# pagmerek/frave

Hardware: AMD Instinct MI355X
Metric: Mpixels/s encode (transform+quant) at 4096x4096 (higher is better)
Workload: dtype u8->i32

## Files before the change

### frave_amd/csrc/fri_hip.cpp

```cpp
#include "fri_hip_internal.hpp"
#include "region_table.hpp"

#include <atomic>
#include <cstdio>
#include <cstdlib>
#include <mutex>
#include <new>
#include <optional>
#include <thread>

#include "search_scaffold.hpp"
#include "solve6.hpp"

using namespace fri;
using namespace fri::host;

void PlanDelete::operator()(fri_hip_plan *p) const { delete p; }

struct fri_hip_multi {
    std::vector<fri_hip_ctx *> ctxs;
    std::vector<fri_hip_plan *> plans;
};

namespace {
// ... 15 lines not shown
    std::vector<float> t(10 * 1024);
    for (int b = 0; b < 10; b++)
        for (uint32_t j = 0; j < 1024; j++) {
            const float x = (float)((j & 1u) ? (int32_t)(j + 1) / -2 : (int32_t)(j / 2));
            t[b * 1024 + j] = std::exp(-std::fabs(x - 0.0f) / width[b]) / (2.0f * width[b]);
        }
    return t;
}

struct Knobs {
    int band_rows = 0, cells_per_tile = 0, cells_per_wg = 0, target_wgs = 0, tile_bytes = 0;
    int ranks = 0;
    std::optional<int> strided_shares;
    std::optional<int> k1_wave;
    int k1_wave_band = 0, k1_wave_wgs = 0;
    bool has_rank_weights = false;
    float rank_weight[4] = {0, 0, 0, 0};
    bool pins_forward = false;
    int batch_share_tiles = 0;
    std::optional<int> inv_shared, inv_strided_shares;
    int inv_band_rows = 0;
    int pred_blocks = 0, hist_blocks = 0, trace = 0, k3_scan = 0;
    int k1_ablate = 0, k2_ablate = 0, k3_ablate = 0, k4_ablate = 0;
    std::optional<int> k1_cached_stores, k1_batch_shares, k4_older_eighths;
};

Knobs read_knobs() {
    Knobs k;
    const char *on = std::getenv("FRI_HIP_TUNING");
    if (!on || on[0] != '1' || on[1] != 0) return k;
    auto env = [](const char *name) { return std::getenv(name); };
    auto pin = [&](const char *name) {
        const char *s = env(name);
        k.pins_forward |= s != nullptr;
        return s;
    };
    auto opt = [](const char *s) { return s ? std::optional<int>(std::atoi(s)) : std::nullopt; };
    auto num = [&](const char *s) { return opt(s).value_or(0); };
    k.band_rows = num(pin("FRI_HIP_BAND_ROWS")), k.cells_per_tile = num(pin("FRI_HIP_CELLS_PER_TILE")), k.cells_per_wg = num(pin("FRI_HIP_CELLS_PER_WG"));
    k.target_wgs = num(pin("FRI_HIP_TARGET_WGS")), k.tile_bytes = num(pin("FRI_HIP_TILE_BYTES")), k.ranks = std::min(num(pin("FRI_HIP_RANKS")), 4);
    k.strided_shares = opt(pin("FRI_HIP_STRIDED_SHARES"));
    k.k1_wave = opt(pin("FRI_HIP_K1_WAVE"));
    k.k1_wave_band = num(pin("FRI_HIP_K1_WAVE_BAND")), k.k1_wave_wgs = num(pin("FRI_HIP_K1_WAVE_WGS"));
    if (const char *s = pin("FRI_HIP_RANK_WEIGHTS")) {
        float *w = k.rank_weight;
        k.has_rank_weights = std::sscanf(s, "%f,%f,%f,%f", &w[0], &w[1], &w[2], &w[3]) == 4;
    }
    k.batch_share_tiles = num(env("FRI_HIP_BATCH_SHARE_TILES"));
    k.inv_shared = opt(env("FRI_HIP_INV_SHARED")), k.inv_strided_shares = opt(env("FRI_HIP_INV_STRIDED_SHARES")), k.inv_band_rows = num(env("FRI_HIP_INV_BAND_ROWS"));
    k.pred_blocks = num(env("FRI_HIP_PRED_BLOCKS")), k.hist_blocks = num(env("FRI_HIP_HIST_BLOCKS")), k.trace = num(env("FRI_HIP_TRACE")), k.k3_scan = num(env("FRI_HIP_K3_SCAN"));
    k.k1_ablate = num(env("FRI_HIP_K1_ABLATE")), k.k2_ablate = num(env("FRI_HIP_K2_ABLATE")), k.k3_ablate = num(env("FRI_HIP_K3_ABLATE")), k.k4_ablate = num(env("FRI_HIP_K4_ABLATE"));
    k.k1_cached_stores = opt(env("FRI_HIP_K1_CACHED_STORES")), k.k1_batch_shares = opt(env("FRI_HIP_K1_BATCH_SHARES")), k.k4_older_eighths = opt(env("FRI_HIP_K4_OLDER_EIGHTHS"));
    return k;
}

int acquire_acc(fri_hip_plan *p, hipStream_t stream, uint32_t n_planes = 1) {
    fri_hip_ctx *c = p->ctx;
    HIP_TRY(c, hipSetDevice(c->device));
// ... 90 lines not shown
            HIP_TRY(c, hipMalloc((void **)s.d_oob.put(), 2 * C * sizeof(unsigned long long)));
            HIP_TRY(c, hipHostMalloc((void **)s.h_oob.put(), 2 * C * sizeof(unsigned long long), hipHostMallocDefault));
            HIP_TRY(c, hipMalloc((void **)s.d_params.put(), C * sizeof(PredictParams)));
            HIP_TRY(c, hipHostMalloc((void **)s.h_params.put(), C * sizeof(PredictParams), hipHostMallocDefault));
        }
    }
    return FRI_HIP_OK;
}


void fill_forward_tiling(DevicePlan &d, const Geometry &g) {
    d.n_tiles = (uint32_t)g.tiles.size(), d.n_wg = (uint32_t)g.wg_tiles.size() - 1, d.n_wg_batch = (uint32_t)g.wg_tiles_batch.size() - 1;
    d.lds_pitch = g.lds_pitch, d.lds_rows = g.lds_rows, d.cells_per_tile = g.cells_per_tile, d.max_tile_cells = g.max_tile_cells;
    d.max_wg_tiles = std::max(g.max_wg_tiles, g.max_wg_tiles_batch), d.max_wg_cells = g.max_wg_cells;
    d.n_wave_wg = g.wave_cells.empty() ? 0u : (uint32_t)g.wave_cells.size() - 1, d.max_wave_wg_cells = g.max_wave_wg_cells;
    if (g.wave_cells.empty()) d.wave_meta = nullptr, d.wave_cells = nullptr;
}
void fill_inverse_tiling(DevicePlan &d, const Geometry &g) {
    fill_forward_tiling(d, g);
    d.wg_tiles_batch = nullptr, d.n_wg_batch = 0, d.max_wg_tiles = g.max_wg_tiles;
    d.wave_meta = nullptr, d.wave_cells = nullptr, d.n_wave_wg = 0, d.max_wave_wg_cells = 0;
    d.inv_group = 1, d.inv_max_wg_tiles = g.max_wg_tiles, d.inv_max_wg_cells = g.max_wg_cells;
}

hipError_t upload_tiling(std::vector<DevMem<void>> &bufs, const Geometry &g, DevicePlan &d, bool inverse) {
    hipError_t e;
    if ((e = upload(bufs, g.tiles, d.tiles)) || (e = upload(bufs, g.tile_cells, d.tile_cells)) || (e = upload(bufs, g.tile_meta, d.tile_meta)) ||
        (e = upload(bufs, g.wg_tiles, d.wg_tiles)) || (!inverse && (e = upload(bufs, g.wg_tiles_batch, d.wg_tiles_batch))))
        return e;
    if (!inverse && !g.wave_cells.empty() && ((e = upload(bufs, g.wave_meta, d.wave_meta)) || (e = upload(bufs, g.wave_cells, d.wave_cells)))) return e;
    inverse ? fill_inverse_tiling(d, g) : fill_forward_tiling(d, g);
    return hipSuccess;
}

int fwd_resident(const Geometry &g, uint32_t channels) {
    DevicePlan d;
// ... 37 lines not shown

constexpr size_t kStridedMaxCells = 200000, kOwnInverseMaxCells = 400000;
constexpr size_t kInvListsMaxBytes = (size_t)256 << 20;

int choose_forward_tiling(uint32_t width, uint32_t height, uint32_t channels, std::optional<int> cus, const Knobs &k, Tiling &t) {
    TilingParams &tp = t.tp;
    tp.band_rows = k.band_rows;
    tp.cells_per_tile = k.cells_per_tile;
    tp.cells_per_wg = k.cells_per_wg;
    tp.batch_share_tiles = k.batch_share_tiles;
    tp.strided_shares = k.strided_shares ? *k.strided_shares > 0 : cus.has_value();
    if (!k.strided_shares && (size_t)width * height / kCell >= kStridedMaxCells) tp.strided_shares = false;
    if (tp.band_rows <= 0 && cus) tp.band_rows = 16;
    tp.tile_buffer_bytes = k.tile_bytes > 0 ? k.tile_bytes : (channels == 1 ? 4 : 6) * 256 * 16;
    set_ranks(tp, k.ranks > 0 ? k.ranks : 4, cus, k);
    if (k.k1_wave.value_or(0) > 0 && cus) tp.wave_ranks = std::min(k.k1_wave_wgs > 0 ? k.k1_wave_wgs : 4, fwd_wave_resident()), tp.wave_band_rows = std::max(k.k1_wave_band, 0);
    for (;;) {
        const std::string err = build_geometry(width, height, channels, tp, t.geo);
        if (!err.empty()) return err == "empty lattice" ? FRI_HIP_ERR_EMPTY_LATTICE : FRI_HIP_ERR_INVALID_ARGUMENT;
        const int resident = fwd_resident(t.geo, channels);
        const size_t F = t.geo.centers.size();
        if (!resident) {
            if (!shrink_tiling(tp, t.geo)) return FRI_HIP_ERR_INVALID_ARGUMENT;
        } else if (cus && !k.strided_shares && tp.strided_shares && F >= kStridedMaxCells) {
            tp.strided_shares = false;
        } else if (cus && k.ranks <= 0 && resident < tp.ranks) {
            set_ranks(tp, resident, cus, k);
        } else if (cus && !t.many_shares && k.target_wgs <= 0 && tp.cells_per_wg <= 0 && F >= 128 * (size_t)(*cus * tp.ranks)) {
            t.many_shares = true;
            tp.target_wgs = (int)(((F / 32 + 1023) / 1024) * 1024);
            for (int i = 0; i < 4; i++) tp.rank_weight[i] = i < tp.ranks ? 1.f : 0.f;
        } else {
            return FRI_HIP_OK;
        }
    }
}

bool choose_inverse_tiling(uint32_t width, uint32_t height, uint32_t channels, std::optional<int> cus, const Knobs &k, const Tiling &fwd, Tiling &inv) {
    if (!cus || (k.inv_shared ? *k.inv_shared > 0 : fwd.geo.centers.size() >= kOwnInverseMaxCells)) return false;
    TilingParams &ti = inv.tp;
    ti = fwd.tp;
    ti.wave_ranks = 0;
    set_ranks(ti, fwd.tp.ranks, cus, k);
    ti.band_rows = k.inv_band_rows > 0 ? k.inv_band_rows : (channels == 1 ? 32 : 16);
    ti.cells_per_tile = k.cells_per_tile;
    ti.cells_per_wg = 0;
    ti.target_wgs = *cus * ti.ranks;
    ti.strided_shares = k.inv_strided_shares ? *k.inv_strided_shares > 0 : k.strided_shares.value_or(1) > 0;
    for (int guard = 0; guard < 64; guard++) {
        if (!build_geometry(width, height, channels, ti, inv.geo).empty()) return false;
        if (fwd_resident(inv.geo, channels) && inv_fits(inv.geo, channels, false)) {
            build_inverse_lists(inv.geo, kInvListsMaxBytes);
            return inv.geo.inv_lists.empty() || inv_fits(inv.geo, channels, true);
        }
        if (!shrink_tiling(ti, inv.geo)) return false;
    }
    return false;
// ... 22 lines not shown
    return resident > 0 && resident >= c.tp.ranks;
}

hipError_t upload_forward_candidate(const fri_hip_plan *p, FwdTiling &c) {
    c.dev = p->dev;
    c.dev.k1_measuring = true;
    return upload_tiling(c.bufs, c.geo, c.dev, false);
}

void adopt_forward_tiling(fri_hip_plan *p, FwdTiling &c) {
    Geometry &g = p->geo;
    g.tiles.swap(c.geo.tiles), g.tile_cells.swap(c.geo.tile_cells), g.tile_meta.swap(c.geo.tile_meta), g.wg_tiles.swap(c.geo.wg_tiles), g.wg_tiles_batch.swap(c.geo.wg_tiles_batch);
    g.max_wg_tiles_batch = c.geo.max_wg_tiles_batch, g.lds_pitch = c.geo.lds_pitch, g.lds_rows = c.geo.lds_rows, g.band_rows = c.geo.band_rows, g.cells_per_tile = c.geo.cells_per_tile;
    g.cells_per_wg = c.geo.cells_per_wg, g.max_tile_cells = c.geo.max_tile_cells, g.max_wg_tiles = c.geo.max_wg_tiles, g.max_wg_cells = c.geo.max_wg_cells;
    g.wave_meta.swap(c.geo.wave_meta), g.wave_cells.swap(c.geo.wave_cells);
    g.wave_band_rows = c.geo.wave_band_rows, g.wave_ranks = c.geo.wave_ranks, g.max_wave_wg_cells = c.geo.max_wave_wg_cells;
    DevicePlan &d = p->dev;
    d.tiles = c.dev.tiles, d.tile_cells = c.dev.tile_cells, d.tile_meta = c.dev.tile_meta, d.wg_tiles = c.dev.wg_tiles, d.wg_tiles_batch = c.dev.wg_tiles_batch;
    d.wave_meta = c.dev.wave_meta, d.wave_cells = c.dev.wave_cells;
    fill_forward_tiling(d, g);
    d.inv_max_wg_tiles = d.max_wg_tiles, d.inv_max_wg_cells = d.max_wg_cells;
    for (auto &b : c.bufs) p->owned.push_back(std::move(b));
    c.bufs.clear();
    p->fwd_tp = c.tp;
    p->fwd_tiling_note = c.label;
}

std::string tiling_label(const TilingParams &tp, const Geometry &g) {
    char b[96];
    if (tp.wave_ranks > 0 && !g.wave_cells.empty()) std::snprintf(b, sizeof b, "wave/band%d/wg%d", g.wave_band_rows, g.wave_ranks);
    else std::snprintf(b, sizeof b, "%s/band%d/cells%d", tp.strided_shares ? "interleaved" : "contiguous", g.band_rows, g.cells_per_tile);
    std::string l = b;
    if (tp.rank_weight[0] > 0) {
        std::snprintf(b, sizeof b, "/w%.2f-%.2f", tp.rank_weight[0], tp.rank_weight[std::max(0, std::min(tp.ranks, 4) - 1)]);
        l += b;
    }
    return l;
}

struct TunedKey {
    int device;
    uint32_t w, h, c;
    bool operator==(const TunedKey &o) const { return device == o.device && w == o.w && h == o.h && c == o.c; }
};
std::mutex g_tuned_mu;
std::vector<std::pair<TunedKey, TilingParams>> g_tuned;

void adopt_cached_forward_tiling(fri_hip_plan *p) {
// ... 170 lines not shown
    if (!out) return FRI_HIP_ERR_INVALID_ARGUMENT;
    *out = nullptr;
    const StaticTables &st = static_tables();
    if (!st.error.empty() || !device_footprint_matches(st)) return FRI_HIP_ERR_INVALID_ARGUMENT;
    std::unique_ptr<fri_hip_plan, PlanDelete> plan(new (std::nothrow) fri_hip_plan);
    if (!plan) return FRI_HIP_ERR_OUT_OF_MEMORY;
    fri_hip_plan *p = plan.get();
    p->ctx = ctx;
    const Knobs k = read_knobs();
    const std::optional<int> cus = ctx ? std::optional<int>(ctx->cu_count) : std::nullopt;
    Tiling fwd, inv;
    if (int rc = choose_forward_tiling(width, height, channels, cus, k, fwd)) return rc;
    p->own_inverse_tiling = choose_inverse_tiling(width, height, channels, cus, k, fwd, inv);
    p->geo = std::move(fwd.geo);
    p->fwd_tp = fwd.tp;
    if (!p->geo.wave_cells.empty()) p->fwd_tiling_note = tiling_label(fwd.tp, p->geo) + " (pinned: FRI_HIP_K1_WAVE)";
    if (p->own_inverse_tiling) {
        p->geo_inv = std::move(inv.geo);
        std::vector<uint32_t>().swap(p->geo_inv.valid_mask), std::vector<int32_t>().swap(p->geo_inv.nbr_cells), std::vector<int32_t>().swap(p->geo_inv.pred_slots);
    } else {
        build_inverse_lists(p->geo, kInvListsMaxBytes);
    }
    if (!ctx) {
        p->dev.n_pred_tiles = p->geo.n_pred_tiles;
        p->dev.pred_blocks = (uint32_t)std::max(k.pred_blocks, 0), p->dev.hist_blocks = (uint32_t)std::max(k.hist_blocks, 0);
        p->dev.k4_older_eighths = k.k4_older_eighths.value_or(0);
        *out = plan.release();
        return FRI_HIP_OK;
    }
    if (hipSetDevice(ctx->device) != hipSuccess) return FRI_HIP_ERR_HIP;
    const Geometry &g = p->geo, &gi = p->inv_geo();
// ... 1035 lines not shown
    }
    for (uint32_t k = 1; k < n_streams; k++) {
        HIP_TRY(c, hipEventRecord(done[k], st[k]));
        HIP_TRY(c, hipStreamWaitEvent(st[0], done[k], 0));
    }
    HIP_TRY(c, hipEventRecord(e1, st[0]));
    HIP_TRY(c, hipEventSynchronize(e1));
    float ms = 0.f;
    HIP_TRY(c, hipEventElapsedTime(&ms, e0, e1));
    *mean_us = (double)ms * 1000.0 / iters;
    return FRI_HIP_OK;
}

static int tune_forward(fri_hip_plan *p, uint32_t launches, std::string &rep) {
    if (!p->fwd_tunable) {
        rep = "{\"tuned\": false, \"kept\": \"" + p->fwd_tiling_note + "\", \"why\": \"tiling pinned by the environment, shared with the inverse kernel, or a many-shares plan\"}";
        return FRI_HIP_OK;
    }
    fri_hip_ctx *c = p->ctx;
    HIP_TRY(c, hipSetDevice(c->device));
    if (!launches) launches = 96;
    const Geometry &g0 = p->geo;
    const bool rgb = g0.channels != 1;
    std::vector<std::unique_ptr<FwdTiling>> cand;
    auto add_tp = [&](const TilingParams &tp) {
        auto t = std::make_unique<FwdTiling>();
        t->tp = tp;
        if (t->tp.cells_per_tile < 0 || t->tp.band_rows < 0) return;
        if (!build_forward_candidate(p, *t)) return;
        t->label = tiling_label(t->tp, t->geo);
        for (const auto &o : cand)
// ... 108 lines not shown
            size_t b2 = best;
            for (size_t k : round2)
                if (cand[k]->us < cand[b2]->us) b2 = k;
            if (cand[b2]->us < cand[best]->us * 0.99) best = b2;
        }
    }
    if (!rgb && g0.width % 16 == 0) {
        const TilingParams w = cand[best]->tp;
        std::vector<size_t> round3{best};
        const size_t n0 = cand.size();
        for (int ranks : {4, 5})
            for (int band : {16, 32, 72, 96, 112, 128}) {
                if (ranks == 5 && band != 32 && band != 96) continue;
                TilingParams tp = w;
                tp.wave_ranks = ranks, tp.wave_band_rows = band;
                add_tp(tp);
                if (band >= (int)g0.height) break;
            }
        for (size_t k = n0; k < cand.size(); k++) {
            HIP_TRY(c, upload_forward_candidate(p, *cand[k]));
            round3.push_back(k);
        }
        if (round3.size() > 1) {
            HIP_TRY(c, measure(round3));
            size_t b3 = best;
            for (size_t k : round3)
                if (cand[k]->us < cand[b3]->us) b3 = k;
            if (cand[b3]->us < cand[best]->us * 0.985) best = b3;
        }
    }
    std::string xcd_note;
    if (hipMalloc((void **)d_stat.put(), 16 * sizeof(unsigned long long)) == hipSuccess) {
        unsigned long long h_stat[16];
        HIP_TRY(c, hipMemsetAsync(d_stat, 0, sizeof h_stat, stream));
        cand[best]->dev.k1_xcd_stat = d_stat;
        const hipError_t e_run = run(*cand[best], launches);
        cand[best]->dev.k1_xcd_stat = nullptr;
        HIP_TRY(c, e_run);
        HIP_TRY(c, hipStreamSynchronize(stream));
        HIP_TRY(c, hipMemcpy(h_stat, d_stat, sizeof h_stat, hipMemcpyDeviceToHost));
        for (int x = 0; x < 8; x++) {
            char b[32];
            std::snprintf(b, sizeof b, "%s%.2f", x ? " " : "", h_stat[2 * x + 1] ? (double)h_stat[2 * x] / (double)h_stat[2 * x + 1] / 100.0 : 0.0);
// ... 34 lines not shown
```

### frave_amd/csrc/geometry.cpp

```cpp
#include "geometry.hpp"

#include <algorithm>
#include <climits>
#include <cstdlib>
#include <cstring>
#include <deque>

namespace fri {

namespace {

constexpr Int2 kLiterals[11] = {{0, 1}, {-1, 1}, {2, 0}, {-3, -1}, {5, -1}, {1, 3}, {-11, -1}, {9, -5}, {13, 7}, {-31, 3}, {5, -17}};

inline Int2 add(Int2 a, Int2 b) { return {a.x + b.x, a.y + b.y}; }
inline Int2 sub(Int2 a, Int2 b) { return {a.x - b.x, a.y - b.y}; }
inline Int2 neg(Int2 a) { return {-a.x, -a.y}; }
inline int floor_div(int a, int b) { return (a >= 0) ? a / b : -((-a + b - 1) / b); }
inline int pos_mod(int a, int m) {
    int r = a % m;
    return r < 0 ? r + m : r;
}

struct LatticeBasis {
    Int2 zl, zmd;
// ... 140 lines not shown
        zmd = add(kLiterals[depth + 1], zl);
    }
    out[0] = zl;
    out[1] = sub(zl, zmd);
    out[2] = neg(zmd);
    out[3] = neg(zl);
    out[4] = sub(zmd, zl);
    out[5] = zmd;
}

static void build_wave_shares(const TilingParams &tp, Geometry &g) {
    const size_t F = g.centers.size();
    const int ranks = std::min(std::max(tp.wave_ranks, 1), 6), tile_ranks = std::min(std::max(tp.ranks, 1), 4);
    const int band_rows = tp.wave_band_rows > 0 ? tp.wave_band_rows : 16;
    const size_t cus = std::max<size_t>(1, (size_t)(tp.target_wgs > 0 ? tp.target_wgs : 1024) / tile_ranks);
    g.wave_band_rows = band_rows, g.wave_ranks = ranks;
    const int cy_min = g.centers.front().y;
    std::vector<int32_t> order(F);
    for (size_t k = 0; k < F; k++) order[k] = (int32_t)k;
    std::sort(order.begin(), order.end(), [&](int32_t l, int32_t r) {
        const int bl = (g.centers[l].y - cy_min) / band_rows, br = (g.centers[r].y - cy_min) / band_rows;
        if (bl != br) return bl < br;
        if (g.centers[l].x != g.centers[r].x) return g.centers[l].x < g.centers[r].x;
        return g.centers[l].y < g.centers[r].y;
    });
    g.wave_meta.resize(F);
    for (size_t k = 0; k < F; k++) g.wave_meta[k] = TileCell{g.centers[order[k]].x, g.centers[order[k]].y, order[k], g.interior[order[k]]};
    const size_t n_wg = std::max<size_t>(1, std::min(cus * ranks, (F + 1) / 2));
    const bool weighted = tp.rank_weight[0] > 0 && tp.rank_weight[tile_ranks - 1] > 0;
    auto weight = [&](size_t rank) {
        if (!weighted || ranks == 1) return 1.0;
        return (double)tp.rank_weight[0] + ((double)tp.rank_weight[tile_ranks - 1] - (double)tp.rank_weight[0]) * (double)rank / (double)(ranks - 1);
    };
    std::vector<double> cum(n_wg + 1, 0.0);
    const size_t q = n_wg >> 3, r = n_wg & 7;
    for (size_t x = 0, sh = 0; x < 8; x++) {
        const size_t n_x = q + (x < r ? 1 : 0);
        for (size_t idx = 0; idx < n_x; idx++, sh++) cum[sh + 1] = cum[sh] + weight(std::min<size_t>((idx * 8 + x) / cus, ranks - 1));
    }
    g.wave_cells.assign(n_wg + 1, 0);
    for (size_t sh = 0; sh <= n_wg; sh++) g.wave_cells[sh] = (int32_t)((double)F * cum[sh] / cum[n_wg] + 0.5);
    g.wave_cells[0] = 0;
    g.wave_cells[n_wg] = (int32_t)F;
    g.max_wave_wg_cells = 0;
    for (size_t sh = 1; sh <= n_wg; sh++) {
        g.wave_cells[sh] = (int32_t)std::min<size_t>(std::max<size_t>((size_t)g.wave_cells[sh], (size_t)g.wave_cells[sh - 1] + 1), F - (n_wg - sh));
        g.max_wave_wg_cells = std::max(g.max_wave_wg_cells, g.wave_cells[sh] - g.wave_cells[sh - 1]);
// ... 354 lines not shown
```

### frave_amd/csrc/geometry.hpp

```cpp
#pragma once
#include <cstdint>
#include <string>
#include <vector>

namespace fri {

struct Int2 {
    int32_t x, y;
};

constexpr int kDepth = 9;
constexpr int kCell = 1 << kDepth;
constexpr int kNbr = 8;

struct StaticTables {
    Int2 literals[11];
    Int2 leaf_off[kCell];
    uint16_t residue_lut[kCell];
    Int2 v9[6];
    Int2 nbr_delta[kNbr];
    uint16_t nbr_table[kCell][6];
    std::string error;
};
const StaticTables &static_tables();
// ... 23 lines not shown
    uint64_t n_valid_leaves = 0;
    std::vector<Int2> centers;
    std::vector<uint8_t> interior;
    std::vector<uint32_t> valid_mask;
    std::vector<int32_t> nbr_cells;
    std::vector<Tile> tiles;
    std::vector<int32_t> tile_cells;
    std::vector<TileCell> tile_meta;
    std::vector<int32_t> wg_tiles;
    std::vector<int32_t> wg_tiles_batch;
    int32_t max_wg_tiles_batch = 0;
    std::vector<TileCell> wave_meta;
    std::vector<int32_t> wave_cells;
    int32_t wave_band_rows = 0, wave_ranks = 0;
    int32_t max_wave_wg_cells = 0;
    std::vector<InvTileLists> inv_lists;
    std::vector<uint16_t> inv_quads, inv_dwords;
    std::vector<uint32_t> inv_parts;
    int32_t inv_rect_bytes = 0;
    int32_t lds_pitch = 0;
    int32_t lds_rows = 0;
    int32_t band_rows = 0, cells_per_tile = 0, cells_per_wg = 0;
    int32_t max_tile_cells = 0;
    int32_t max_wg_tiles = 0;
    int32_t max_wg_cells = 0;
    std::vector<int32_t> pred_slots;
    uint32_t n_pred_tiles = 0;
};

constexpr int32_t kPredSlotInterior = 0x40000000;
constexpr int kPredBlock = 4;
constexpr int kPredSide = kPredBlock + 2;
constexpr int kPredSlots = kPredSide * kPredSide;

struct TilingParams {
    int band_rows = 0, cells_per_tile = 0;
    int target_wgs = 0;
    int cells_per_wg = 0;
    float rank_weight[4] = {0, 0, 0, 0};
    int ranks = 4;
    int tile_buffer_bytes = 0;
    int batch_share_tiles = 0;
    int wave_ranks = 0, wave_band_rows = 0;
    bool strided_shares = false;
};

std::string build_geometry(uint32_t width, uint32_t height, uint32_t channels, const TilingParams &tp, Geometry &out);
void build_inverse_lists(Geometry &g, size_t max_bytes);

}
```

### frave_amd/csrc/k1_forward.hip

```cpp
#include "device_common.hpp"

namespace fri {
namespace {

constexpr int kFwdThreads = 256;
constexpr int kFwdWaves = kFwdThreads / 64;

constexpr int kMaxPairsPerWave = 2;
constexpr int kMaxItemsPerTile = 2 * kMaxPairsPerWave * kFwdWaves;
constexpr int kMaxChunksPerThread = 6;

struct FwdArgs {
    const uint8_t *pixels;
    size_t pixel_stride;
    int32_t *coefs;
    size_t coef_stride;
    const Tile *tiles;
    const TileCell *tile_meta;
    const int32_t *wg_tiles;
    uint32_t n_wg;
    int32_t width, height;
    uint32_t F;
    int32_t pitch;
    int32_t meta_off;
    int32_t buf_bytes;
    uint32_t cpr, cpr_magic;
    int32_t q_identity;
    int32_t ablate;
    unsigned long long *trace;
    unsigned long long *xcd_stat;
    QMatrix q;
};

__device__ __forceinline__ uint32_t pk_low(uint32_t l, uint32_t r, uint32_t x) { return __builtin_amdgcn_lerp(l, r, x >> 15); }
__device__ __forceinline__ void pk_pair(uint32_t l, uint32_t r, int &dA, int &dB, uint32_t &s) {
    s = pk_low(l, r, l - r);
    dA = (int)(l & 0xFFFFu) - (int)(r & 0xFFFFu);
    dB = (int)(l >> 16) - (int)(r >> 16);
}
__device__ __forceinline__ void unpack_x(uint32_t x, int &dA, int &dB) {
    dA = (int)(short)(x & 0xFFFFu);
    dB = (int)(x + 0x8000u) >> 16;
}
// ... 514 lines not shown

constexpr int kWavePitch = 160, kWaveRows = 21, kWaveItemBytes = 64;
constexpr int kWaveSlab = kWaveRows * kWavePitch;
constexpr int kWaveItemChunks = kWaveRows * 4;
constexpr int kWaveLoads = 3;
constexpr int kWaveLdsBytes = 2 * kFwdWaves * kWaveSlab;
constexpr int kWaveMaxWgCells = 64 * kFwdWaves;
typedef u32x4 __attribute__((address_space(3))) *LdsQuadPtr;

struct WaveChunks {
    int row[kWaveLoads], k16[kWaveLoads];
    bool item_b[kWaveLoads], used[kWaveLoads];
    uint32_t lds_off[kWaveLoads];
};

template <bool QID, bool MEASURE = false>
__global__ void __launch_bounds__(kFwdThreads) fwd_wave_kernel(const FwdArgs a) {
    __shared__ __attribute__((aligned(16))) uint8_t slabs[kWaveLdsBytes];
    const int tid = threadIdx.x, lane = tid & 63;
    const int wave = __builtin_amdgcn_readfirstlane(tid >> 6);
    const uint32_t wg = xcd_contiguous_share(blockIdx.x, a.n_wg);
    const int cb = a.wg_tiles[wg], ce = a.wg_tiles[wg + 1];
    const unsigned long long t_entry = a.xcd_stat ? wall_clock64() : 0ull;
    const int wg_pairs = (ce - cb + 1) >> 1;
    const int n_pairs = wg_pairs > wave ? (wg_pairs - wave + kFwdWaves - 1) / kFwdWaves : 0;
    if (n_pairs > 0) {
        const uint8_t *img = a.pixels + (size_t)blockIdx.y * a.pixel_stride;
        int32_t *coefs = a.coefs + (size_t)blockIdx.y * a.coef_stride;
        const int mine = cb + 2 * (wave + kFwdWaves * (lane >> 1)) + (lane & 1);
        const i32x4 rec = reinterpret_cast<const i32x4 *>(a.tile_meta)[min(mine, ce - 1)];
        const uint32_t slab0 = (uint32_t)(uintptr_t)(__attribute__((address_space(3))) uint8_t *)slabs + (uint32_t)wave * (2u * kWaveSlab);

        WaveChunks ch;
#pragma unroll
        for (int c = 0; c < kWaveLoads; c++) {
            const int s = lane + 64 * c;
            ch.used[c] = s < 2 * kWaveItemChunks;
            ch.item_b[c] = s >= kWaveItemChunks;
            const int w = ch.item_b[c] ? s - kWaveItemChunks : s;
            ch.row[c] = ch.used[c] ? w >> 2 : 0;
            ch.k16[c] = 16 * (w & 3);
// ... 13 lines not shown
            for (int c = 0; c < kWaveLoads; c++) {
                const int x = (ch.item_b[c] ? xB : xA) + ch.k16[c], y = (ch.item_b[c] ? cyB : cyA) - 8 + ch.row[c];
                const bool inside = wanted && ch.used[c] && (uint32_t)x < (uint32_t)a.width && (uint32_t)y < (uint32_t)a.height;
                st[c] = *reinterpret_cast<const u32x4 *>(img + (inside ? (uint32_t)y * (uint32_t)a.width + (uint32_t)x : 0u));
            }
        };
        auto commit = [&](uint32_t slab) {
#pragma unroll
            for (int c = 0; c < kWaveLoads; c++) *(LdsQuadPtr)(uintptr_t)(slab + ch.lds_off[c]) = st[c];
        };
        issue(0, true);
        commit(slab0);

        for (int i = 0; i < n_pairs; i++) {
            const uint32_t cur = slab0 + (uint32_t)(i & 1) * kWaveSlab, nxt = slab0 + (uint32_t)((i & 1) ^ 1) * kWaveSlab;
            issue(min(i + 1, n_pairs - 1), i + 1 < n_pairs);
            __builtin_amdgcn_s_setprio(3);
            const int cxA = __builtin_amdgcn_readlane(rec.x, 2 * i), cyA = __builtin_amdgcn_readlane(rec.y, 2 * i);
            const int cxB = __builtin_amdgcn_readlane(rec.x, 2 * i + 1), cyB = __builtin_amdgcn_readlane(rec.y, 2 * i + 1);
            const uint32_t offA = (uint32_t)__builtin_amdgcn_readlane(rec.z, 2 * i) * kCell, offB = (uint32_t)__builtin_amdgcn_readlane(rec.z, 2 * i + 1) * kCell;
            const int interior = __builtin_amdgcn_readlane(rec.w, 2 * i) & __builtin_amdgcn_readlane(rec.w, 2 * i + 1);
            const bool store_b = cb + 2 * (wave + kFwdWaves * i) + 1 < ce;
            const int baseA = (int)cur + ((cxA - 15) & 15), baseB = (int)cur + kWaveItemBytes + ((cxB - 15) & 15);
            const int wbA[3] = {baseA + wo[0], baseA + wo[1], baseA + wo[2]}, wbB[3] = {baseB + wo[0], baseB + wo[1], baseB + wo[2]};
            uint32_t wA[3], wB[3], maskA = 0xFFu, maskB = 0xFFu;
            fetch_windows(wbA, wA);
            fetch_windows(wbB, wB);
            if (interior == 0) {
                maskA = maskB = 0;
#pragma unroll
// ... 16 lines not shown
            leaf[7] = pair_bytes<2>(wA[2], wB[2]);
            int resA[8], resB[8];
            fwd_wave_pk(leaf, lane, resA, resB);
            __builtin_amdgcn_s_setprio(1);
            uint32_t valid = 0xFFFFFFFFu;
            if (interior == 0) valid = validity_tree_pk(maskA | (maskB << 16), lane);
            commit(nxt);
            __builtin_amdgcn_s_setprio(0);
            if (__builtin_amdgcn_readfirstlane(valid == 0xFFFFFFFFu ? 1 : 0) && __all(valid == 0xFFFFFFFFu)) {
                store_item<0, false, QID, true>(coefs, offA, lane, resA, valid, a);
                if (store_b) store_item<1, false, QID, true>(coefs, offB, lane, resB, valid, a);
            } else {
                store_item<0, true, QID, true>(coefs, offA, lane, resA, valid, a);
                if (store_b) store_item<1, true, QID, true>(coefs, offB, lane, resB, valid, a);
            }
        }
    }
    if (a.xcd_stat && tid == 0) {
        const uint32_t xcc = __builtin_amdgcn_s_getreg((3 << 11) | 20) & 7u;
        (void)__hip_atomic_fetch_add(a.xcd_stat + 2 * xcc, wall_clock64() - t_entry, __ATOMIC_RELAXED, __HIP_MEMORY_SCOPE_AGENT);
        (void)__hip_atomic_fetch_add(a.xcd_stat + 2 * xcc + 1, 1ull, __ATOMIC_RELAXED, __HIP_MEMORY_SCOPE_AGENT);
    }
}


}

const void *pick_forward_ycbcr(bool edge, bool fast, bool small, bool qid, bool plain, bool measure, bool c16);
#ifndef FRI_K1_YCBCR_INSTANCES

static size_t fwd_meta_offset(const DevicePlan &p) { return ((size_t)p.lds_pitch * p.lds_rows + 15) & ~(size_t)15; }
static size_t fwd_buf_bytes(const DevicePlan &p) { return fwd_meta_offset(p) + (size_t)p.max_tile_cells * sizeof(TileCell); }
// ... 44 lines not shown
    a.cpr_magic = (uint32_t)(((1ull << 32) + a.cpr - 1) / a.cpr);
    a.q = q;
    a.q_identity = 1;
    for (int i = 0; i <= 9; i++) a.q_identity &= (q.q[i] == 1);
    a.ablate = p.k1_ablate;
    a.trace = p.trace;
    a.xcd_stat = p.k1_xcd_stat;
    const size_t lds = fwd_lds_bytes(p);
    const dim3 grid(a.n_wg, n_images), block(kFwdThreads);
    const size_t img_bytes = (size_t)p.width * p.height * p.channels;
    const bool edge = (reinterpret_cast<uintptr_t>(pixels) & 15) || (img_bytes & 15) || (n_images > 1 && (pixel_stride & 15));
    const bool fast = !edge && (((size_t)p.width * p.channels) & 15) == 0;
    const bool small = fwd_chunks(p) <= 4 * (size_t)kFwdThreads;
    const bool rct = p.rct && p.channels == 3;
    const bool ycc = p.ycc && p.channels == 3;
    if (fast && !plain && !coefs16 && n_images < 8 && !p.trace && !p.k1_ablate && fwd_wave_fits(p)) {
        a.tile_meta = p.wave_meta;
        a.wg_tiles = p.wave_cells;
        a.n_wg = p.n_wave_wg;
        void (*wk)(FwdArgs) = a.q_identity ? (p.k1_measuring ? fwd_wave_kernel<true, true> : fwd_wave_kernel<true>) : fwd_wave_kernel<false>;
        (void)hipGetLastError();
        hipLaunchKernelGGL(wk, dim3(a.n_wg, n_images), block, 0, stream, a);
        return hipGetLastError();
    }
    void (*kern)(FwdArgs);
#define FRI_PICK_T(CH, E, FA, N, QI, R) (plain ? fwd_transform_quant_kernel<CH, E, FA, N, QI, false, false, false, R> : fwd_transform_quant_kernel<CH, E, FA, N, QI, true, false, false, R>)
#define FRI_PICK_Q(CH, E, FA, N, R) (a.q_identity ? FRI_PICK_T(CH, E, FA, N, true, R) : FRI_PICK_T(CH, E, FA, N, false, R))
#define FRI_PICK_N(CH, E, FA, R) (small ? FRI_PICK_Q(CH, E, FA, 4, R) : FRI_PICK_Q(CH, E, FA, kMaxChunksPerThread, R))
#define FRI_PICK(CH, R) (edge ? FRI_PICK_N(CH, true, false, R) : fast ? FRI_PICK_N(CH, false, true, R) : FRI_PICK_N(CH, false, false, R))
    kern = p.channels == 1 ? FRI_PICK(1, false) : rct ? FRI_PICK(3, true) : FRI_PICK(3, false);
    if (p.k1_measuring && !edge && !plain && a.q_identity) {
#define FRI_PICK_M(CH, R) (fast ? (small ? fwd_transform_quant_kernel<CH, false, true, 4, true, true, true, false, R> : fwd_transform_quant_kernel<CH, false, true, kMaxChunksPerThread, true, true, true, false, R>) \
                                : (small ? fwd_transform_quant_kernel<CH, false, false, 4, true, true, true, false, R> : fwd_transform_quant_kernel<CH, false, false, kMaxChunksPerThread, true, true, true, false, R>))
        kern = p.channels == 1 ? FRI_PICK_M(1, false) : rct ? FRI_PICK_M(3, true) : FRI_PICK_M(3, false);
#undef FRI_PICK_M
// ... 27 lines not shown
```

### frave_amd/csrc/kernels.hpp

```cpp
#pragma once
#include <hip/hip_runtime_api.h>

#include <cstddef>
#include <cstdint>

#include "geometry.hpp"

namespace fri {

struct DevicePlan {
    const Tile *tiles = nullptr;
    const int32_t *tile_cells = nullptr;
    const TileCell *tile_meta = nullptr;
    const int32_t *wg_tiles = nullptr;
    const int32_t *wg_tiles_batch = nullptr;
    uint32_t n_wg_batch = 0;
    uint32_t n_wg = 0;
    const TileCell *wave_meta = nullptr;
    const int32_t *wave_cells = nullptr;
    uint32_t n_wave_wg = 0;
    int32_t max_wave_wg_cells = 0;
    int32_t max_tile_cells = 0;
    bool covers_image = false;
    int32_t max_wg_tiles = 0;
    int32_t max_wg_cells = 0;
    int32_t inv_group = 1;
    int32_t inv_max_wg_tiles = 0, inv_max_wg_cells = 0;
    const Int2 *centers = nullptr;
    const uint8_t *interior = nullptr;
    const uint32_t *valid_mask = nullptr;
    const int32_t *nbr_cells = nullptr;
    const uint16_t *nbr_table = nullptr;
    const uint32_t *gather_off = nullptr;
    const uint16_t *pair_pos = nullptr;
    const uint16_t *heap_of_pos = nullptr;
    const uint32_t *halo_list = nullptr;
// ... 145 lines not shown

hipError_t launch_split_tiles_rgba(const uint8_t *rgba, uint32_t width, uint32_t height, uint32_t tile_w, uint32_t tile_h, bool clean, uint8_t *colour_tiles, uint8_t *alpha_tiles,
                                   hipStream_t stream);
hipError_t launch_merge_tiles_rgba_region(const uint8_t *colour_tiles, const uint8_t *alpha_tiles, uint32_t width, uint32_t height, uint32_t tile_w, uint32_t tile_h, uint32_t x,
                                          uint32_t y, uint32_t w, uint32_t h, uint8_t *region, hipStream_t stream);

void build_lf_deltas(const uint16_t *nbr_table, int8_t *out );
void build_gather_tables(const uint16_t *nbr_table, uint32_t *gather_off , uint16_t *pair_pos , uint16_t *heap_of_pos );
void build_halo_list(const uint16_t *nbr_table, const uint16_t *pair_pos, uint32_t *out );
size_t fwd_lds_bytes(const DevicePlan &p);
size_t inv_lds_bytes(const DevicePlan &p);
bool device_footprint_matches(const StaticTables &st);
bool fwd_plan_fits(const DevicePlan &p);
bool fwd_wave_fits(const DevicePlan &p);
int fwd_wave_resident();
constexpr size_t kInvListPad = 2048;
bool inv_plan_fits(const DevicePlan &p, bool with_lists);

}
```

Baseline: 936,700.

## Add paced wave-kernel variant and autotune pacing and wave rank weights

```diff
diff --git a/frave_amd/csrc/fri_hip.cpp b/frave_amd/csrc/fri_hip.cpp
--- a/frave_amd/csrc/fri_hip.cpp
+++ b/frave_amd/csrc/fri_hip.cpp
@@ -53,6 +53,7 @@
     std::optional<int> strided_shares;
     std::optional<int> k1_wave;
     int k1_wave_band = 0, k1_wave_wgs = 0;
+    int k1_wave_pace = 0;
     bool has_rank_weights = false;
     float rank_weight[4] = {0, 0, 0, 0};
     bool pins_forward = false;
@@ -81,6 +82,7 @@
     k.strided_shares = opt(pin("FRI_HIP_STRIDED_SHARES"));
     k.k1_wave = opt(pin("FRI_HIP_K1_WAVE"));
     k.k1_wave_band = num(pin("FRI_HIP_K1_WAVE_BAND")), k.k1_wave_wgs = num(pin("FRI_HIP_K1_WAVE_WGS"));
+    k.k1_wave_pace = num(pin("FRI_HIP_K1_WAVE_PACE"));
     if (const char *s = pin("FRI_HIP_RANK_WEIGHTS")) {
         float *w = k.rank_weight;
         k.has_rank_weights = std::sscanf(s, "%f,%f,%f,%f", &w[0], &w[1], &w[2], &w[3]) == 4;
@@ -201,12 +203,13 @@
     d.lds_pitch = g.lds_pitch, d.lds_rows = g.lds_rows, d.cells_per_tile = g.cells_per_tile, d.max_tile_cells = g.max_tile_cells;
     d.max_wg_tiles = std::max(g.max_wg_tiles, g.max_wg_tiles_batch), d.max_wg_cells = g.max_wg_cells;
     d.n_wave_wg = g.wave_cells.empty() ? 0u : (uint32_t)g.wave_cells.size() - 1, d.max_wave_wg_cells = g.max_wave_wg_cells;
+    d.wave_pace_ticks = g.wave_cells.empty() ? 0u : std::min((uint32_t)std::max(g.wave_pace_ticks, 0), kWavePaceMaxTicks);
     if (g.wave_cells.empty()) d.wave_meta = nullptr, d.wave_cells = nullptr;
 }
 void fill_inverse_tiling(DevicePlan &d, const Geometry &g) {
     fill_forward_tiling(d, g);
     d.wg_tiles_batch = nullptr, d.n_wg_batch = 0, d.max_wg_tiles = g.max_wg_tiles;
-    d.wave_meta = nullptr, d.wave_cells = nullptr, d.n_wave_wg = 0, d.max_wave_wg_cells = 0;
+    d.wave_meta = nullptr, d.wave_cells = nullptr, d.n_wave_wg = 0, d.max_wave_wg_cells = 0, d.wave_pace_ticks = 0;
     d.inv_group = 1, d.inv_max_wg_tiles = g.max_wg_tiles, d.inv_max_wg_cells = g.max_wg_cells;
 }
 
@@ -274,7 +277,9 @@
     if (tp.band_rows <= 0 && cus) tp.band_rows = 16;
     tp.tile_buffer_bytes = k.tile_bytes > 0 ? k.tile_bytes : (channels == 1 ? 4 : 6) * 256 * 16;
     set_ranks(tp, k.ranks > 0 ? k.ranks : 4, cus, k);
-    if (k.k1_wave.value_or(0) > 0 && cus) tp.wave_ranks = std::min(k.k1_wave_wgs > 0 ? k.k1_wave_wgs : 4, fwd_wave_resident()), tp.wave_band_rows = std::max(k.k1_wave_band, 0);
+    const bool wave_pinned = k.k1_wave ? *k.k1_wave > 0 : k.k1_wave_pace > 0;
+    if (wave_pinned && cus) tp.wave_ranks = std::min(k.k1_wave_wgs > 0 ? k.k1_wave_wgs : 4, fwd_wave_resident()), tp.wave_band_rows = std::max(k.k1_wave_band, 0);
+    if (wave_pinned && cus && k.k1_wave_pace > 0) tp.wave_pace_ticks = (int)std::min<uint32_t>((uint32_t)k.k1_wave_pace, kWavePaceMaxTicks);
     for (;;) {
         const std::string err = build_geometry(width, height, channels, tp, t.geo);
         if (!err.empty()) return err == "empty lattice" ? FRI_HIP_ERR_EMPTY_LATTICE : FRI_HIP_ERR_INVALID_ARGUMENT;
@@ -300,7 +305,7 @@
     if (!cus || (k.inv_shared ? *k.inv_shared > 0 : fwd.geo.centers.size() >= kOwnInverseMaxCells)) return false;
     TilingParams &ti = inv.tp;
     ti = fwd.tp;
-    ti.wave_ranks = 0;
+    ti.wave_ranks = 0, ti.wave_pace_ticks = 0;
     set_ranks(ti, fwd.tp.ranks, cus, k);
     ti.band_rows = k.inv_band_rows > 0 ? k.inv_band_rows : (channels == 1 ? 32 : 16);
     ti.cells_per_tile = k.cells_per_tile;
@@ -353,7 +358,7 @@
     g.max_wg_tiles_batch = c.geo.max_wg_tiles_batch, g.lds_pitch = c.geo.lds_pitch, g.lds_rows = c.geo.lds_rows, g.band_rows = c.geo.band_rows, g.cells_per_tile = c.geo.cells_per_tile;
     g.cells_per_wg = c.geo.cells_per_wg, g.max_tile_cells = c.geo.max_tile_cells, g.max_wg_tiles = c.geo.max_wg_tiles, g.max_wg_cells = c.geo.max_wg_cells;
     g.wave_meta.swap(c.geo.wave_meta), g.wave_cells.swap(c.geo.wave_cells);
-    g.wave_band_rows = c.geo.wave_band_rows, g.wave_ranks = c.geo.wave_ranks, g.max_wave_wg_cells = c.geo.max_wave_wg_cells;
+    g.wave_band_rows = c.geo.wave_band_rows, g.wave_ranks = c.geo.wave_ranks, g.max_wave_wg_cells = c.geo.max_wave_wg_cells, g.wave_pace_ticks = c.geo.wave_pace_ticks;
     DevicePlan &d = p->dev;
     d.tiles = c.dev.tiles, d.tile_cells = c.dev.tile_cells, d.tile_meta = c.dev.tile_meta, d.wg_tiles = c.dev.wg_tiles, d.wg_tiles_batch = c.dev.wg_tiles_batch;
     d.wave_meta = c.dev.wave_meta, d.wave_cells = c.dev.wave_cells;
@@ -367,10 +372,18 @@
 
 std::string tiling_label(const TilingParams &tp, const Geometry &g) {
     char b[96];
-    if (tp.wave_ranks > 0 && !g.wave_cells.empty()) std::snprintf(b, sizeof b, "wave/band%d/wg%d", g.wave_band_rows, g.wave_ranks);
+    const bool wave = tp.wave_ranks > 0 && !g.wave_cells.empty();
+    if (wave) std::snprintf(b, sizeof b, "wave/band%d/wg%d", g.wave_band_rows, g.wave_ranks);
     else std::snprintf(b, sizeof b, "%s/band%d/cells%d", tp.strided_shares ? "interleaved" : "contiguous", g.band_rows, g.cells_per_tile);
     std::string l = b;
-    if (tp.rank_weight[0] > 0) {
+    if (wave && g.wave_pace_ticks > 0) {
+        std::snprintf(b, sizeof b, "/pace%d", (g.wave_pace_ticks + 5) / 10);
+        l += b;
+    }
+    if (wave && tp.wave_weight[0] > 0) {
+        std::snprintf(b, sizeof b, "/w%.2f-%.2f", tp.wave_weight[0], tp.wave_weight[1]);
+        l += b;
+    } else if (tp.rank_weight[0] > 0) {
         std::snprintf(b, sizeof b, "/w%.2f-%.2f", tp.rank_weight[0], tp.rank_weight[std::max(0, std::min(tp.ranks, 4) - 1)]);
         l += b;
     }
@@ -571,7 +584,7 @@
     p->own_inverse_tiling = choose_inverse_tiling(width, height, channels, cus, k, fwd, inv);
     p->geo = std::move(fwd.geo);
     p->fwd_tp = fwd.tp;
-    if (!p->geo.wave_cells.empty()) p->fwd_tiling_note = tiling_label(fwd.tp, p->geo) + " (pinned: FRI_HIP_K1_WAVE)";
+    if (!p->geo.wave_cells.empty()) p->fwd_tiling_note = tiling_label(fwd.tp, p->geo) + (fwd.tp.wave_pace_ticks > 0 ? " (pinned: FRI_HIP_K1_WAVE_PACE)" : " (pinned: FRI_HIP_K1_WAVE)");
     if (p->own_inverse_tiling) {
         p->geo_inv = std::move(inv.geo);
         std::vector<uint32_t>().swap(p->geo_inv.valid_mask), std::vector<int32_t>().swap(p->geo_inv.nbr_cells), std::vector<int32_t>().swap(p->geo_inv.pred_slots);
@@ -1637,7 +1650,14 @@
 
 static int tune_forward(fri_hip_plan *p, uint32_t launches, std::string &rep) {
     if (!p->fwd_tunable) {
-        rep = "{\"tuned\": false, \"kept\": \"" + p->fwd_tiling_note + "\", \"why\": \"tiling pinned by the environment, shared with the inverse kernel, or a many-shares plan\"}";
+        rep = "{\"tuned\": false, \"kept\": \"" + p->fwd_tiling_note + "\", \"why\": \"tiling pinned by the environment, shared with the inverse kernel, or a many-shares plan\"";
+        if (p->dev.n_wave_wg > 0) {
+            const int max_pairs = ((p->dev.max_wave_wg_cells + 1) / 2 + 3) / 4;
+            rep += ", \"wave_form\": {\"shares\": " + std::to_string(p->dev.n_wave_wg) + ", \"max_pairs_per_wave\": " + std::to_string(max_pairs) + ", \"pace_ticks\": " +
+                   std::to_string(p->dev.wave_pace_ticks) + ", \"pace_step_cycles\": " + std::to_string(64 * kWavePaceSleep) + ", \"pace_max_steps\": " + std::to_string(kWavePaceMaxSteps) +
+                   ", \"pace_max_ticks\": " + std::to_string(kWavePaceMaxTicks) + "}";
+        }
+        rep += "}";
         return FRI_HIP_OK;
     }
     fri_hip_ctx *c = p->ctx;
@@ -1776,6 +1796,7 @@
                 if (ranks == 5 && band != 32 && band != 96) continue;
                 TilingParams tp = w;
                 tp.wave_ranks = ranks, tp.wave_band_rows = band;
+                tp.wave_pace_ticks = 0, tp.wave_weight[0] = tp.wave_weight[1] = 0.f;
                 add_tp(tp);
                 if (band >= (int)g0.height) break;
             }
@@ -1789,6 +1810,37 @@
             for (size_t k : round3)
                 if (cand[k]->us < cand[b3]->us) b3 = k;
             if (cand[b3]->us < cand[best]->us * 0.985) best = b3;
+        }
+        size_t bw = cand.size();
+        for (size_t k : round3)
+            if (cand[k]->tp.wave_ranks > 0 && cand[k]->tp.wave_pace_ticks == 0 && (bw == cand.size() || cand[k]->us < cand[bw]->us)) bw = k;
+        if (bw != cand.size()) {
+            const TilingParams ww = cand[bw]->tp;
+            const double t_w = cand[bw]->us;
+            std::vector<size_t> round4{best};
+            if (bw != best) round4.push_back(bw);
+            const size_t n1 = cand.size();
+            static const float cuts[3][2] = {{0.f, 0.f}, {1.15f, 0.85f}, {1.f, 1.f}};
+            for (const auto &cut : cuts) {
+                if (cut[0] == 1.f && !(ww.rank_weight[0] > 0)) continue;
+                for (double ratio : {0.70, 0.75, 0.80, 0.85}) {
+                    TilingParams tp = ww;
+                    tp.wave_weight[0] = cut[0], tp.wave_weight[1] = cut[1];
+                    tp.wave_pace_ticks = (int)std::min<uint32_t>(kWavePaceMaxTicks, 10u * (uint32_t)std::max(1.0, ratio * t_w * 10.0 + 0.5));
+                    add_tp(tp);
+                }
+            }
+            for (size_t k = n1; k < cand.size(); k++) {
+                HIP_TRY(c, upload_forward_candidate(p, *cand[k]));
+                round4.push_back(k);
+            }
+            if (cand.size() > n1) {
+                HIP_TRY(c, measure(round4));
+                size_t b4 = best;
+                for (size_t k = n1; k < cand.size(); k++)
+                    if (cand[k]->us < cand[b4]->us) b4 = k;
+                if (cand[b4]->us < cand[best]->us * 0.985) best = b4;
+            }
         }
     }
     std::string xcd_note;
diff --git a/frave_amd/csrc/geometry.cpp b/frave_amd/csrc/geometry.cpp
--- a/frave_amd/csrc/geometry.cpp
+++ b/frave_amd/csrc/geometry.cpp
@@ -178,7 +178,7 @@
     const int ranks = std::min(std::max(tp.wave_ranks, 1), 6), tile_ranks = std::min(std::max(tp.ranks, 1), 4);
     const int band_rows = tp.wave_band_rows > 0 ? tp.wave_band_rows : 16;
     const size_t cus = std::max<size_t>(1, (size_t)(tp.target_wgs > 0 ? tp.target_wgs : 1024) / tile_ranks);
-    g.wave_band_rows = band_rows, g.wave_ranks = ranks;
+    g.wave_band_rows = band_rows, g.wave_ranks = ranks, g.wave_pace_ticks = std::max(tp.wave_pace_ticks, 0);
     const int cy_min = g.centers.front().y;
     std::vector<int32_t> order(F);
     for (size_t k = 0; k < F; k++) order[k] = (int32_t)k;
@@ -191,10 +191,12 @@
     g.wave_meta.resize(F);
     for (size_t k = 0; k < F; k++) g.wave_meta[k] = TileCell{g.centers[order[k]].x, g.centers[order[k]].y, order[k], g.interior[order[k]]};
     const size_t n_wg = std::max<size_t>(1, std::min(cus * ranks, (F + 1) / 2));
-    const bool weighted = tp.rank_weight[0] > 0 && tp.rank_weight[tile_ranks - 1] > 0;
+    const bool own = tp.wave_weight[0] > 0 && tp.wave_weight[1] > 0;
+    const double w_first = own ? tp.wave_weight[0] : tp.rank_weight[0], w_last = own ? tp.wave_weight[1] : tp.rank_weight[tile_ranks - 1];
+    const bool weighted = w_first > 0 && w_last > 0;
     auto weight = [&](size_t rank) {
         if (!weighted || ranks == 1) return 1.0;
-        return (double)tp.rank_weight[0] + ((double)tp.rank_weight[tile_ranks - 1] - (double)tp.rank_weight[0]) * (double)rank / (double)(ranks - 1);
+        return w_first + (w_last - w_first) * (double)rank / (double)(ranks - 1);
     };
     std::vector<double> cum(n_wg + 1, 0.0);
     const size_t q = n_wg >> 3, r = n_wg & 7;
diff --git a/frave_amd/csrc/geometry.hpp b/frave_amd/csrc/geometry.hpp
--- a/frave_amd/csrc/geometry.hpp
+++ b/frave_amd/csrc/geometry.hpp
@@ -61,6 +61,7 @@
     std::vector<int32_t> wave_cells;
     int32_t wave_band_rows = 0, wave_ranks = 0;
     int32_t max_wave_wg_cells = 0;
+    int32_t wave_pace_ticks = 0;
     std::vector<InvTileLists> inv_lists;
     std::vector<uint16_t> inv_quads, inv_dwords;
     std::vector<uint32_t> inv_parts;
@@ -89,6 +90,8 @@
     int tile_buffer_bytes = 0;
     int batch_share_tiles = 0;
     int wave_ranks = 0, wave_band_rows = 0;
+    int wave_pace_ticks = 0;
+    float wave_weight[2] = {0, 0};
     bool strided_shares = false;
 };
 
diff --git a/frave_amd/csrc/k1_forward.hip b/frave_amd/csrc/k1_forward.hip
--- a/frave_amd/csrc/k1_forward.hip
+++ b/frave_amd/csrc/k1_forward.hip
@@ -27,6 +27,7 @@
     uint32_t cpr, cpr_magic;
     int32_t q_identity;
     int32_t ablate;
+    uint32_t pace_ticks;
     unsigned long long *trace;
     unsigned long long *xcd_stat;
     QMatrix q;
@@ -571,17 +572,23 @@
     uint32_t lds_off[kWaveLoads];
 };
 
-template <bool QID, bool MEASURE = false>
+template <bool QID, bool MEASURE = false, bool PACED = false>
 __global__ void __launch_bounds__(kFwdThreads) fwd_wave_kernel(const FwdArgs a) {
     __shared__ __attribute__((aligned(16))) uint8_t slabs[kWaveLdsBytes];
     const int tid = threadIdx.x, lane = tid & 63;
     const int wave = __builtin_amdgcn_readfirstlane(tid >> 6);
     const uint32_t wg = xcd_contiguous_share(blockIdx.x, a.n_wg);
     const int cb = a.wg_tiles[wg], ce = a.wg_tiles[wg + 1];
+    trace_stamp(a.trace, wg, 0, tid);
     const unsigned long long t_entry = a.xcd_stat ? wall_clock64() : 0ull;
     const int wg_pairs = (ce - cb + 1) >> 1;
     const int n_pairs = wg_pairs > wave ? (wg_pairs - wave + kFwdWaves - 1) / kFwdWaves : 0;
     if (n_pairs > 0) {
+        uint32_t pace_entry = 0, pace_step = 0, pace_due = 0;
+        if constexpr (PACED) {
+            pace_entry = (uint32_t)wall_clock64();
+            pace_step = (a.pace_ticks << 8) / (uint32_t)n_pairs;
+        }
         const uint8_t *img = a.pixels + (size_t)blockIdx.y * a.pixel_stride;
         int32_t *coefs = a.coefs + (size_t)blockIdx.y * a.coef_stride;
         const int mine = cb + 2 * (wave + kFwdWaves * (lane >> 1)) + (lane & 1);
@@ -625,6 +632,13 @@
 
         for (int i = 0; i < n_pairs; i++) {
             const uint32_t cur = slab0 + (uint32_t)(i & 1) * kWaveSlab, nxt = slab0 + (uint32_t)((i & 1) ^ 1) * kWaveSlab;
+            if constexpr (PACED) {
+                if (i > 0) {
+                    pace_due += pace_step;
+#pragma nounroll
+                    for (int step = 0; step < kWavePaceMaxSteps && (uint32_t)wall_clock64() - pace_entry < (pace_due >> 8); step++) __builtin_amdgcn_s_sleep(kWavePaceSleep);
+                }
+            }
             issue(min(i + 1, n_pairs - 1), i + 1 < n_pairs);
             __builtin_amdgcn_s_setprio(3);
             const int cxA = __builtin_amdgcn_readlane(rec.x, 2 * i), cyA = __builtin_amdgcn_readlane(rec.y, 2 * i);
@@ -671,8 +685,10 @@
                 store_item<0, true, QID, true>(coefs, offA, lane, resA, valid, a);
                 if (store_b) store_item<1, true, QID, true>(coefs, offB, lane, resB, valid, a);
             }
-        }
-    }
+            trace_stamp(a.trace, wg, 1 + i, tid);
+        }
+    }
+    trace_exit(a.trace, wg, tid);
     if (a.xcd_stat && tid == 0) {
         const uint32_t xcc = __builtin_amdgcn_s_getreg((3 << 11) | 20) & 7u;
         (void)__hip_atomic_fetch_add(a.xcd_stat + 2 * xcc, wall_clock64() - t_entry, __ATOMIC_RELAXED, __HIP_MEMORY_SCOPE_AGENT);
@@ -747,11 +763,15 @@
     const bool small = fwd_chunks(p) <= 4 * (size_t)kFwdThreads;
     const bool rct = p.rct && p.channels == 3;
     const bool ycc = p.ycc && p.channels == 3;
-    if (fast && !plain && !coefs16 && n_images < 8 && !p.trace && !p.k1_ablate && fwd_wave_fits(p)) {
+    if (fast && !plain && !coefs16 && n_images < 8 && (!p.trace || p.n_wave_wg <= p.n_wg) && !p.k1_ablate && fwd_wave_fits(p)) {
         a.tile_meta = p.wave_meta;
         a.wg_tiles = p.wave_cells;
         a.n_wg = p.n_wave_wg;
         void (*wk)(FwdArgs) = a.q_identity ? (p.k1_measuring ? fwd_wave_kernel<true, true> : fwd_wave_kernel<true>) : fwd_wave_kernel<false>;
+        if (p.wave_pace_ticks > 0 && n_images == 1) {
+            a.pace_ticks = p.wave_pace_ticks < kWavePaceMaxTicks ? p.wave_pace_ticks : kWavePaceMaxTicks;
+            wk = a.q_identity ? (p.k1_measuring ? fwd_wave_kernel<true, true, true> : fwd_wave_kernel<true, false, true>) : fwd_wave_kernel<false, false, true>;
+        }
         (void)hipGetLastError();
         hipLaunchKernelGGL(wk, dim3(a.n_wg, n_images), block, 0, stream, a);
         return hipGetLastError();
diff --git a/frave_amd/csrc/kernels.hpp b/frave_amd/csrc/kernels.hpp
--- a/frave_amd/csrc/kernels.hpp
+++ b/frave_amd/csrc/kernels.hpp
@@ -20,6 +20,7 @@
     const int32_t *wave_cells = nullptr;
     uint32_t n_wave_wg = 0;
     int32_t max_wave_wg_cells = 0;
+    uint32_t wave_pace_ticks = 0;
     int32_t max_tile_cells = 0;
     bool covers_image = false;
     int32_t max_wg_tiles = 0;
@@ -195,6 +196,8 @@
 bool fwd_plan_fits(const DevicePlan &p);
 bool fwd_wave_fits(const DevicePlan &p);
 int fwd_wave_resident();
+constexpr int kWavePaceSleep = 4, kWavePaceMaxSteps = 16;
+constexpr uint32_t kWavePaceMaxTicks = 1u << 16;
 constexpr size_t kInvListPad = 2048;
 bool inv_plan_fits(const DevicePlan &p, bool with_lists);
 
```

After: 999,000 (median of 6 runs). 1.07x the previous value.
